# ga1i13o/DiffewS

Measured on AMD Instinct MI355X. Metric: few-shot episodes/sec (512x512, 1-shot, SD-2 UNet), higher is better.
Workload: dtype bf16; 1 GPU; SD-2.1 UNet + SD VAE, 512x512, 1-shot, 4 episodes/GPU/step (BASELINE.json configs[1]); nshot=1, resolution=512, parallelism=episode-sharded x1, hip_graph=True, residual_dtype=bf16, graph_owner=pipeline.run_episodes(captured=True)

## Files before the change

### diffews_amd/_lib.py

```python
import ctypes as C
import os

_HERE = os.path.dirname(os.path.abspath(__file__))
LIB_PATH = os.environ.get("DFW_LIB") or os.path.join(_HERE, "libdiffews_hip.so")

BF16, F16 = 0, 1
FILTER_BILINEAR, FILTER_BICUBIC = 0, 1
OUT_T, OUT_F32, OUT_NCHW_F32 = 0, 1, 2
ACT_NONE, ACT_SILU, ACT_CLAMP1 = 0, 1, 2

_vp, _i32, _i64, _f32, _sz = C.c_void_p, C.c_int32, C.c_int64, C.c_float, C.c_size_t


class GemmArgs(C.Structure):
    _fields_ = [("A", _vp), ("W", _vp), ("C", _vp), ("bias", _vp), ("rowbias", _vp), ("residual", _vp),
                ("workspace", _vp), ("workspace_bytes", _sz), ("a_elems", _i64), ("w_elems", _i64),
                ("M", _i32), ("N", _i32), ("K", _i32), ("lda", _i32), ("ldc", _i32), ("ldr", _i32), ("ld_rowbias", _i32),
                ("taps", _i32), ("Cin", _i32), ("Hi", _i32), ("Wi", _i32), ("Ho", _i32), ("Wo", _i32),
                ("stride", _i32), ("pad", _i32), ("ups", _i32), ("rows_per_img", _i32),
                ("out_scale", _f32), ("act", _i32), ("geglu", _i32), ("out_mode", _i32), ("splitk", _i32),
                ("batch", _i32), ("strideA", _i64), ("strideW", _i64), ("strideC", _i64), ("dtype", _i32),
                ("gn_partial", _vp), ("gn_groups", _i32),
                ("colscale", _f32), ("colscale_n", _i32), ("residual_f32", _i32), ("W_blocked", _vp)]


class FsaArgs(C.Structure):
    _fields_ = [("q", _vp), ("k", _vp), ("v", _vp), ("k_bank", _vp), ("v_bank", _vp), ("out", _vp),
                ("batch", _i32), ("heads", _i32), ("n_q", _i32), ("n_kv", _i32), ("n_bank", _i32), ("nshot", _i32),
                ("ldq", _i32), ("ldk", _i32), ("ldv", _i32), ("ldkb", _i32), ("ldvb", _i32), ("ldo", _i32),
                ("q_bs", _i64), ("k_bs", _i64), ("v_bs", _i64), ("kb_bs", _i64), ("vb_bs", _i64), ("o_bs", _i64),
                ("scale", _f32), ("dtype", _i32), ("n_plain", _i32), ("q_prescaled", _i32), ("lse", _vp),
                ("workspace", _vp), ("workspace_bytes", _sz), ("bank_shared", _i32)]


class XattnArgs(C.Structure):
    _fields_ = [("q", _vp), ("k", _vp), ("v", _vp), ("out", _vp),
                ("batch", _i32), ("heads", _i32), ("n_q", _i32), ("L", _i32),
                ("ldq", _i32), ("ldk", _i32), ("ldv", _i32), ("ldo", _i32),
                ("q_bs", _i64), ("k_bs", _i64), ("v_bs", _i64), ("o_bs", _i64),
                ("scale", _f32), ("dtype", _i32)]


class GroupNormArgs(C.Structure):
    _fields_ = [("x", _vp), ("y", _vp), ("gamma", _vp), ("beta", _vp), ("stats_ws", _vp), ("stats_ws_bytes", _sz),
                ("B", _i32), ("HW", _i32), ("C", _i32), ("groups", _i32), ("ldx", _i32), ("ldy", _i32),
                ("eps", _f32), ("silu", _i32), ("dtype", _i32), ("pre_partial", _vp), ("pre_chunks", _i32),
                ("x_f32", _i32)]


class LayerNormArgs(C.Structure):
    _fields_ = [("x", _vp), ("y", _vp), ("gamma", _vp), ("beta", _vp),
                ("rows", _i32), ("C", _i32), ("ldx", _i32), ("ldy", _i32), ("eps", _f32), ("dtype", _i32),
                ("x_f32", _i32)]


class ConvSmallArgs(C.Structure):
    _fields_ = [("x", _vp), ("W", _vp), ("bias", _vp), ("y", _vp),
                ("B", _i32), ("Cin", _i32), ("H", _i32), ("Wd", _i32), ("Cout", _i32), ("taps", _i32), ("ldy", _i32),
# ... 99 lines not shown
                ("q_bs", _i64), ("kv_bs", _i64), ("o_bs", _i64), ("dq_bs", _i64), ("dkv_bs", _i64),
                ("scale", _f32), ("dtype", _i32), ("workspace", _vp), ("workspace_bytes", _sz), ("delta_bytes", _sz)]


class VattnArgs(C.Structure):
    _fields_ = [("q", _vp), ("k", _vp), ("v", _vp), ("out", _vp),
                ("batch", _i32), ("n", _i32), ("head_dim", _i32), ("q_prescaled", _i32),
                ("ldq", _i32), ("ldk", _i32), ("ldv", _i32), ("ldo", _i32),
                ("q_bs", _i64), ("k_bs", _i64), ("v_bs", _i64), ("o_bs", _i64), ("dtype", _i32)]


class AdamWArgs(C.Structure):
    _fields_ = [("param", _vp), ("grad", _vp), ("exp_avg", _vp), ("exp_avg_sq", _vp), ("grad_sumsq", _vp), ("n", _i64),
                ("lr", _f32), ("beta1", _f32), ("beta2", _f32), ("eps", _f32), ("weight_decay", _f32), ("max_grad_norm", _f32),
                ("step", _i32), ("shadow", _vp), ("shadow_dtype", _i32), ("found_inf", _vp)]


class Config(C.Structure):
    _fields_ = [("conv_patch", _i32), ("big_kernels", _i32), ("big_bm", _i32), ("big_bn", _i32), ("big_bk", _i32),
                ("gemm_bm", _i32), ("gemm_bn", _i32), ("fsa_key_split", _i32),
                ("fsa_force_splits", _i32), ("big_min_tiles", _i32), ("k8", _i32)]


SYMBOLS = {
    "dfw_configure": (_i32, [C.POINTER(Config)]),
    "dfw_get_config": (None, [C.POINTER(Config)]),
    "dfw_version": (_i32, []),
    "dfw_error_string": (C.c_char_p, [_i32]),
    "dfw_graph_memset_nodes": (_i32, [_vp, C.POINTER(_i32)]),
    "dfw_gemm": (_i32, [C.POINTER(GemmArgs), _vp]),
    "dfw_gemm_workspace_bytes": (_sz, [C.POINTER(GemmArgs)]),
    "dfw_gemm_kernel_name": (_i32, [C.POINTER(GemmArgs), C.c_char_p, _sz]),
    "dfw_gemm_gn_chunks": (_i32, [C.POINTER(GemmArgs)]),
    "dfw_fsa_attention": (_i32, [C.POINTER(FsaArgs), _vp]),
    "dfw_fsa_workspace_bytes": (_sz, [C.POINTER(FsaArgs)]),
    "dfw_fsa_kernel_name": (_i32, [C.POINTER(FsaArgs), C.c_char_p, _sz]),
    "dfw_fsa_attention_sets": (_i32, [C.POINTER(FsaArgs), _i32, _vp]),
    "dfw_fsa_sets_kernel_name": (_i32, [C.POINTER(FsaArgs), _i32, C.c_char_p, _sz]),
    "dfw_fsa_attention_ragged": (_i32, [C.POINTER(FsaArgs), C.POINTER(_i32), _i32, _i32, _vp]),
    "dfw_fsa_ragged_kernel_name": (_i32, [C.POINTER(FsaArgs), C.POINTER(_i32), _i32, _i32, C.c_char_p, _sz]),
    "dfw_fsa_ragged_workspace_bytes": (_sz, [C.POINTER(FsaArgs), C.POINTER(_i32), _i32, _i32]),
    "dfw_fsa_attention_routed": (_i32, [C.POINTER(FsaArgs), _vp, C.POINTER(_i32), _i32, _i32, _vp]),
    "dfw_fsa_routed_kernel_name": (_i32, [C.POINTER(FsaArgs), _i32, _i32, C.c_char_p, _sz]),
    "dfw_fsa_routed_workspace_bytes": (_sz, [C.POINTER(FsaArgs), _i32, _i32]),
    "dfw_cross_attention": (_i32, [C.POINTER(XattnArgs), _vp]),
    "dfw_vae_attention": (_i32, [C.POINTER(VattnArgs), _vp]),
    "dfw_groupnorm": (_i32, [C.POINTER(GroupNormArgs), _vp]),
    "dfw_groupnorm_workspace_bytes": (_sz, [C.POINTER(GroupNormArgs)]),
    "dfw_layernorm": (_i32, [C.POINTER(LayerNormArgs), _vp]),
    "dfw_conv_small": (_i32, [C.POINTER(ConvSmallArgs), _vp]),
    "dfw_conv_small_gn_chunks": (_i32, [C.POINTER(ConvSmallArgs)]),
    "dfw_conv_small_kernel_name": (_i32, [C.POINTER(ConvSmallArgs), C.c_char_p, _sz]),
    "dfw_softmax_rows": (_i32, [_vp, _vp, _i64, _i32, _f32, _i32, _vp]),
    "dfw_softmax_groups": (_i32, [_vp, _vp, _i64, _i32, _i32, _i32, _i32, _vp]),
    "dfw_transpose": (_i32, [_vp, _vp, _i32, _i32, _i32, _i32, _vp]),
    "dfw_concat_channels": (_i32, [_vp, _vp, _vp, _i64, _i32, _i32, _i32, _vp]),
    "dfw_convert_f32": (_i32, [_vp, _vp, _i64, _i32, _vp]),
    "dfw_zero": (_i32, [_vp, _i64, _vp]),
    "dfw_split_f32": (_i32, [_vp, _vp, _vp, _i64, _i32, _vp]),
    "dfw_timestep_embedding": (_i32, [_vp, _vp, _i32, _i32, _i32, _f32, _i32, _vp]),
    "dfw_seg_postprocess": (_i32, [_vp, _vp, _vp, _vp, _vp, _i32, _i32, _i32, _f32, _vp]),
    "dfw_seg_postprocess_ex": (_i32, [_vp, _vp, _vp, _vp, _vp, _i32, _i32, _i32, _f32, _f32, _i32, _vp]),
    "dfw_seg_labels": (_i32, [_vp, _vp, _vp, _vp, _vp, _i32, _i32, _i32, _i32, _f32, _f32, _i32, _vp]),
    "dfw_seg_labels_cand": (_i32, [_vp, _vp, _vp, C.POINTER(_i32), _vp, _vp, _vp, _vp, _i32, _i32, _i32, _i32, _i32, _f32, _f32,
                                   _vp]),
    "dfw_meter_update": (_i32, [_vp, _vp, _vp, _vp, _i32, _i32, _vp]),
# ... 82 lines not shown
```

### diffews_amd/csrc/gemm8.hip

```cpp
#include "gemm_common.h"
#include <type_traits>

namespace dfw {

template <typename T, bool CONV, int BN>
__global__ __launch_bounds__(512, 2) void gemm8_kernel(const GemmP p) {
  constexpr int BM = 256, HT = 16384;
  constexpr bool N160 = BN == 160;
  static_assert(!(N160 && CONV), "the 256 x 160 tile is instantiated for Linear shapes only");
  constexpr int WH = BN / 128;
  constexpr int WGN = N160 ? 2 : BN / 64, WGM = 8 / WGN;
  constexpr int NBW = N160 ? 5 : 4;
  constexpr int WTM = BM / WGM, MB6 = WTM / 16, MH = MB6 / 2;
  constexpr int WDMA = N160 ? 3 : 2 * WH;
  constexpr int WB160 = 65536, WS160 = 24576;
  constexpr int STG = N160 ? WB160 + 2 * WS160 : (2 + WH) * 32768;
  extern __shared__ __attribute__((aligned(16))) char smem[];
  const int tid = threadIdx.x, lane = tid & 63;
  const int wave = __builtin_amdgcn_readfirstlane(tid >> 6);
  const int wr = wave >> 2;
  const int wm = wave / WGN, wc = wave % WGN;
  const uint32_t lds0 = lds_addr(smem);

  const int ntiles = p.ntm * p.ntn;
  const int nxb = gridDim.x >> 3, xcd = blockIdx.x & 7;
  const int Q = (ntiles + 7) >> 3;
  const int t_end = min(ntiles, (xcd + 1) * Q);
  const int tile0 = xcd * Q + (blockIdx.x >> 3);
  if (tile0 >= t_end) return;
  const int my_tiles = (t_end - tile0 + nxb - 1) / nxb;
  const int nkt = p.K >> 6;
  const int cpt = p.Cin >> 6;

  const int z = blockIdx.y;
  const char* Ab = p.A;
  const char* Wb = p.W;
  char* Cb = p.C;
  if (p.batch > 1) {
    Ab += (size_t)z * p.strideA * sizeof(T);
    Wb += (size_t)z * p.strideW * sizeof(T);
    Cb += (size_t)z * p.strideC * sizeof(T);
  }
  const u32x4 ra = make_srd(Ab, p.a_bytes);
  const u32x4 rw = make_srd(Wb, p.w_bytes);

  auto tile_coords = [&](int t) -> TileC {
    TileC c;
    const int tn = t % p.ntn, tm = t / p.ntn;
    c.m0 = tm * BM;
    c.n0 = tn * BN;
    c.img = 0; c.oy0 = 0; c.ox0 = 0;
    if constexpr (CONV) {
      c.img = tm / p.tpi;
      const int t2 = tm - c.img * p.tpi, tyi = t2 / p.tpr, txi = t2 - tyi * p.tpr;
      c.oy0 = tyi << 4;
      c.ox0 = txi << 4;
    }
    return c;
  };
  auto row_to_m = [&](const TileC& c, int r) -> int {
    if constexpr (CONV) return (c.img * p.Ho + c.oy0 + (r >> 4)) * p.Wo + c.ox0 + (r & 15);
    else return c.m0 + r;
  };

  const int lrow = lane >> 3;
  const int kc = (lane & 7) ^ ((((wave & 1) << 2) + (lane >> 4)) & 7);
  const unsigned limH = p.ups ? 2 * p.Hi : p.Hi, limW = p.ups ? 2 * p.Wi : p.Wi;
  const int ush = p.ups ? 1 : 0;
  int a_kt = 0, a_ti = 0;
  bool a_live = true;
  uint32_t a_v0 = 0;
  int a_m = 0, a_ix0 = 0;
  int a_iy0 = 0;
  uint32_t a_pix = 0;
  auto a_setup = [&](const TileC& c) {
    if constexpr (!CONV) {
      a_m = c.m0 + wave * 8 + lrow;
      a_v0 = (uint32_t)(((size_t)a_m * p.lda + kc * 8) * sizeof(T));
    } else {
      a_iy0 = (c.oy0 + (wave >> 1)) * p.stride - p.pad;
      a_ix0 = (c.ox0 + (wave & 1) * 8 + lrow) * p.stride - p.pad;
      a_pix = (uint32_t)c.img * (uint32_t)(p.Hi * p.Wi);
    }
  };
  auto a_advance = [&]() {
    if (++a_kt == nkt) {
      a_kt = 0;
      if (++a_ti < my_tiles) a_setup(tile_coords(tile0 + a_ti * nxb));
      else a_live = false;
    }
  };
  auto issue_a = [&](int buf) __attribute__((always_inline)) {
    int ky = 0, kx = 0, cc = 0;
    if constexpr (CONV) {
      cc = a_kt / 9;
      const int tap = a_kt - cc * 9;
      ky = tap / 3;
      kx = tap - ky * 3;
    }
#pragma unroll
    for (int h = 0; h < 2; ++h) {
      const uint32_t dst = lds0 + (uint32_t)(h * 32768 + buf * HT) + (uint32_t)wave * 1024u;
#pragma unroll
      for (int j = 0; j < 2; ++j) {
        uint32_t off;
        if constexpr (!CONV) {
          const int dr = h * 128 + j * 64;
          off = (a_m + dr < p.M && a_live) ? a_v0 + (uint32_t)dr * (uint32_t)p.lda * (uint32_t)sizeof(T) + (uint32_t)a_kt * 128u : kOOB;
        } else {
          int iy = a_iy0 + (h * 8 + j * 4) * p.stride + ky, ix = a_ix0 + kx;
          const bool ok = (unsigned)iy < limH && (unsigned)ix < limW && a_live;
          iy >>= ush;
          ix >>= ush;
          off = ok ? ((a_pix + (uint32_t)(iy * p.Wi + ix)) * (uint32_t)p.lda + (uint32_t)(cc * 64 + kc * 8)) * (uint32_t)sizeof(T) : kOOB;
        }
        dma16(ra, off, dst + j * 8192);
      }
    }
    a_advance();
  };
  int w_kt = 0, w_ti = 0;
  bool w_live = true;
  uint32_t w_v0 = 0;
  int w_n = 0;
  auto w_setup = [&](const TileC& c) {
    w_n = c.n0 + wave * 8 + lrow;
    w_v0 = (uint32_t)(((size_t)w_n * p.K + kc * 8) * sizeof(T));
  };
  auto issue_w = [&](int buf) __attribute__((always_inline)) {
    uint32_t koff = (uint32_t)w_kt * 128u;
    if constexpr (CONV) {
      const int cc = w_kt / 9, tap = w_kt - cc * 9;
      koff = (uint32_t)(tap * p.Cin + cc * 64) * (uint32_t)sizeof(T);
    }
    if constexpr (N160) {
      const uint32_t dst = lds0 + (uint32_t)(WB160 + buf * WS160) + (uint32_t)wave * 1024u;
#pragma unroll
      for (int j = 0; j < 3; ++j) {
        const uint32_t off = w_v0 + (uint32_t)(j * 64) * (uint32_t)p.K * (uint32_t)sizeof(T) + koff;
        const bool ok = w_live && (j < 2 || wave < 4);
        dma16(rw, ok ? off : kOOB, dst + j * 8192);
      }
    }
#pragma unroll
    for (int h = 0; h < (N160 ? 0 : WH); ++h) {
      const uint32_t dst = lds0 + (uint32_t)((2 + h) * 32768 + buf * HT) + (uint32_t)wave * 1024u;
#pragma unroll
      for (int j = 0; j < 2; ++j) {
        const uint32_t off = w_v0 + (uint32_t)(h * 128 + j * 64) * (uint32_t)p.K * (uint32_t)sizeof(T) + koff;
        bool ok = w_live;
        if constexpr (BN == 128) ok = ok && (w_n + j * 64 < p.N);
        dma16(rw, ok ? off : kOOB, dst + j * 8192);
      }
    }
    if (++w_kt == nkt) {
      w_kt = 0;
      if (++w_ti < my_tiles) {
        if (p.ntn > 1) w_setup(tile_coords(tile0 + w_ti * nxb));
      } else w_live = false;
    }
  };

  uint32_t ab0, ab1, wb0, wb1;
  {
    const int l15 = lane & 15, l4 = lane >> 4;
    const uint32_t fb = (uint32_t)(l15 * 128 + ((l4 ^ (l15 >> 1)) << 4));
    ab0 = (uint32_t)(wr * 32768 + (wm % (WGM / 2)) * WTM * 128) + fb;
    ab1 = ab0 ^ 64u;
    if constexpr (N160) wb0 = (uint32_t)(WB160 + wc * 80 * 128) + fb;
    else wb0 = (uint32_t)((2 + (wc >> 1)) * 32768 + (wc & 1) * 64 * 128) + fb;
    wb1 = wb0 ^ 64u;
  }
  const uint32_t wbase160 = wb0;

  f32x4 acc6[MB6][NBW];
  typename Tr<T>::v8 fa[MH][2], fw0[2][2], fw1[2][2], fw4[2];
  auto zero6 = [&]() __attribute__((always_inline)) {
#pragma unroll
    for (int i = 0; i < MB6; ++i)
#pragma unroll
      for (int j = 0; j < NBW; ++j) acc6[i][j] = f32x4{0.f, 0.f, 0.f, 0.f};
  };
  auto bar = [&]() __attribute__((always_inline)) {
    __builtin_amdgcn_sched_barrier(0);
    __builtin_amdgcn_s_barrier();
    asm volatile("" ::: "memory");
    __builtin_amdgcn_sched_barrier(0);
  };
  auto lgkm0 = [&]() __attribute__((always_inline)) {
    asm volatile("s_waitcnt lgkmcnt(0)" ::: "memory");
    __builtin_amdgcn_sched_barrier(0);
// ... 145 lines not shown
      if (p.gn_partial) {
        const int cp = lane & 31, rh = lane >> 5;
#pragma unroll
        for (int t = 0; t < 16; ++t) {
          const int r = rh * 16 + t;
          const uint32_t w2 = *(const uint32_t*)(stg + r * 128 + (((cp >> 2) ^ (r & 7)) << 4) + (cp & 3) * 4);
          typename Tr<T>::v4 pr = __builtin_bit_cast(typename Tr<T>::v4, i32x2{(int)w2, 0});
          const float a0 = (float)pr[0], a1 = (float)pr[1];
          gs0 += a0; gq0 += a0 * a0;
          gs1 += a1; gq1 += a1 * a1;
        }
      }
      const int c16 = lane & 7;
#pragma unroll
      for (int t = 0; t < 4; ++t) {
        const int r = (lane >> 3) + 8 * t;
        const int m2 = row_to_m(c, wm * WTM + i * 32 + r);
        const i32x4 val = *(const i32x4*)(stg + r * 128 + ((c16 ^ (r & 7)) << 4));
        if (m2 < p.M)
          *(i32x4*)(Cb + ((size_t)m2 * p.ldc + c.n0 + wc * 64 + c16 * 8) * sizeof(T)) = val;
      }
    }
    if (p.gn_partial) {
      float s2 = gs0 + gs1, q2 = gq0 + gq1;
      s2 += __shfl_xor(s2, 32, 64);
      q2 += __shfl_xor(q2, 32, 64);
      const int cpg = p.N / p.gn_groups, ppg = cpg >> 1;
      for (int o = 1; o < ppg; o <<= 1) {
        s2 += __shfl_xor(s2, o, 64);
        q2 += __shfl_xor(q2, o, 64);
      }
      const int cp = lane & 31;
      if (lane < 32 && (cp & (ppg - 1)) == 0) {
        const int tm = tile_id / p.ntn;
        const int chunk = (tm - c.img * p.tpi) * WGM + wm;
        const int grp = (c.n0 + wc * 64 + 2 * cp) / cpg;
        float* o2 = p.gn_partial + (((size_t)c.img * p.gn_chunks + chunk) * p.gn_groups + grp) * 2;
        o2[0] = s2;
        o2[1] = q2;
      }
    }
  };

  TileC ct = tile_coords(tile0);
  a_setup(ct);
  w_setup(ct);
  issue_w(0);
  issue_a(0);
  issue_w(1);
  wait_vm<WDMA>();
  bar();
  if (wr == 1) bar();
  zero6();
  int kt = 0, ti = 0, buf = 0;
  const int total = my_tiles * nkt;
#pragma unroll 1
  for (int g = 0; g < total; ++g) {
    read_a(0);
    read_w(fw0, 0);
    read_w(fw1, 1);
    if constexpr (N160) read_w4();
    issue_a(buf ^ 1);
    lgkm0();
    bar();
    __builtin_amdgcn_s_setprio(1);
    mfmas(0, 0, fw0);
    mfmas(0, 1, fw1);
    if constexpr (N160) mfmas4(0);
// ... 54 lines not shown
    (void)hipFuncSetAttribute((const void*)kfn, hipFuncAttributeMaxDynamicSharedMemorySize, (int)lds);
    hipLaunchKernelGGL(kfn, grid, dim3(512), lds, st, q);
  } else if constexpr (BN != 160) {
    auto kfn = gemm8_kernel<T, true, BN>;
    (void)hipFuncSetAttribute((const void*)kfn, hipFuncAttributeMaxDynamicSharedMemorySize, (int)lds);
    hipLaunchKernelGGL(kfn, grid, dim3(512), lds, st, q);
  } else {
    return DFW_ESHAPE;
  }
  DFW_CHECK_LAUNCH();
  return 0;
}

bool gemm8_eligible(const GemmP& p, int bn) {
  if (!cfg().k8 || p.out_mode != DFW_OUT_T || p.res_f32) return false;
  if ((p.K % 64) != 0 || (p.Cin % 64) != 0 || p.K / 64 < 2) return false;
  if (bn == 256) return (p.N % 256) == 0;
  return bn == 128 && (p.N % 64) == 0 && cfg().k8 >= 2;
}

bool gemm8_n160_eligible(const GemmP& p) {
  if (!cfg().k8 || !cfg().big_kernels || p.taps != 1 || p.out_mode != DFW_OUT_T || p.res_f32 || p.geglu || p.act != DFW_ACT_NONE) return false;
  if (p.batch > 1 || p.splitk > 1 || (p.N % 160) != 0 || (p.N % 128) == 0 || (p.K % 64) != 0 || p.K / 64 < 2) return false;
  if ((p.ldc % 8) != 0 || ((uintptr_t)p.C & 15)) return false;
  return (long long)((p.M + 255) / 256) * (p.N / 160) >= cfg().big_min_tiles;
}

int launch_gemm8(const GemmP& p, const GemmPlan& pl, hipStream_t st) {
  if (pl.bn == 160) return DFW_BY_DTYPE(p, launch8<T, 160>(p, pl, st));
  if (pl.bn == 256) return DFW_BY_DTYPE(p, launch8<T, 256>(p, pl, st));
  return DFW_BY_DTYPE(p, launch8<T, 128>(p, pl, st));
}

}
```

### diffews_amd/csrc/gemm_common.h

```cpp
#pragma once
#include "common.h"

namespace dfw {

struct GemmP {
  const char* A; const char* W; char* C;
  const char* Wblk;
  const float* bias; const float* rowbias; const char* residual; float* partial;
  uint32_t a_bytes, w_bytes;
  int M, N, K, lda, ldc, ldr, ldrb;
  int taps, Cin, Hi, Wi, Ho, Wo, stride, pad, ups, rows_per_img;
  float out_scale;
  float cs; int cs_n;
  int act, geglu, out_mode, splitk, batch;
  int res_f32;
  long long strideA, strideW, strideC;
  int nk, cpt, ntn, ntm;
  int plan_bm, plan_bn, dtype_bf16;
  float* gn_partial; int gn_groups, gn_chunks;
  int conv_chunk_major;
  int tw, tw_log2, tpr, tpi;
};

template <typename T, bool RF32 = false>
// ... 163 lines not shown
  }
  __device__ __forceinline__ void store(const GemmP& p, float* out, int n_w0, int lane) {
    const int cpg = p.N / p.gn_groups;
#pragma unroll
    for (int j = 0; j < 4; ++j) {
#pragma unroll
      for (int o = 1; o < 16; o <<= 1) {
        s[j] += __shfl_xor(s[j], o, 64);
        q[j] += __shfl_xor(q[j], o, 64);
      }
      if (cpg >= 8) { s[j] += __shfl_xor(s[j], 16, 64); q[j] += __shfl_xor(q[j], 16, 64); }
      if (cpg >= 16) { s[j] += __shfl_xor(s[j], 32, 64); q[j] += __shfl_xor(q[j], 32, 64); }
    }
    if (cpg >= 32) { s[0] += s[1]; q[0] += q[1]; s[2] += s[3]; q[2] += q[3]; }
    if (cpg >= 64) { s[0] += s[2]; q[0] += q[2]; }
    const int l15 = lane & 15, l4 = lane >> 4;
    if (l15 != 0) return;
    const int lstep = cpg >= 16 ? 4 : cpg / 4;
    if (l4 % lstep) return;
    const int jstep = cpg >= 64 ? 4 : (cpg >= 32 ? 2 : 1);
#pragma unroll
    for (int j = 0; j < 4; ++j) {
      if (j % jstep) continue;
      const int grp = (n_w0 + j * 16 + 4 * l4) / cpg;
      out[grp * 2] = s[j];
      out[grp * 2 + 1] = q[j];
    }
  }
};

struct TileC {
  int m0, n0;
  int img, oy0, ox0;
};

enum class GemmKernel { Tile, Big, K8, Patch, Patch8 };
struct GemmPlan {
  GemmKernel kernel;
  int bm, bn, bk, splitk;
  int gn_chunks;
  bool f32o, rf32;
};

#define DFW_BY_DTYPE(p, ...) \
  ((p).dtype_bf16 ? [&] { using T = __bf16; return __VA_ARGS__; }() : [&] { using T = _Float16; return __VA_ARGS__; }())

}
```

### diffews_amd/csrc/misc.hip

```cpp
#include "common.h"
#include <stdio.h>
#include <stdlib.h>

namespace dfw {

struct CsP {
  const float* x; const float* W; const float* bias; char* y;
  int B, Cin, H, Wd, Cout, taps, ldy, out_mode;
  float in_scale, out_scale;
  int iters;
  float* gn_partial; int gn_groups, gn_chunks;
  long long ybs;
  const float* x1; const float* x2; int b0, b1;
};

__device__ __forceinline__ const float* cs_image(const CsP& p, int b) {
  const size_t per = (size_t)p.Cin * p.H * p.Wd;
  if (p.x1 == nullptr || b < p.b0) return p.x + (size_t)b * per;
  if (b < p.b1) return p.x1 + (size_t)(b - p.b0) * per;
  return p.x2 + (size_t)(b - p.b1) * per;
}

template <typename T>
__global__ __launch_bounds__(256) void conv_small_kernel(const CsP p) {
// ... 888 lines not shown
        const int c = count_memset_nodes(child, total, depth + 1);
        if (c < 0) { free(nodes); return -1; }
        cnt += c;
      }
    }
  }
  free(nodes);
  return cnt;
}

extern "C" int dfw_graph_memset_nodes(void* graph, int32_t* n_nodes) {
  if (!graph) return DFW_EINVAL;
  if (n_nodes) *n_nodes = 0;
  const int c = count_memset_nodes((hipGraph_t)graph, n_nodes, 0);
  return c < 0 ? DFW_EINVAL : c;
}

static const dfw_config kDefaultCfg = {3, 1, 0, 0, 0, 0, 0, 1, 0, 192, 3};
static dfw_config g_cfg = kDefaultCfg;
namespace dfw { const dfw_config& cfg() { return g_cfg; } }

extern "C" int dfw_configure(const dfw_config* c) {
  if (!c) { g_cfg = kDefaultCfg; return 0; }
  if (c->conv_patch < 0 || c->conv_patch > 4 || c->fsa_force_splits < 0 || c->big_min_tiles < 1 || c->k8 < 0 || c->k8 > 3) return DFW_EINVAL;
  if (c->gemm_bm && !((c->gemm_bm == 128 && (c->gemm_bn == 128 || c->gemm_bn == 64)) || (c->gemm_bm == 64 && c->gemm_bn == 64))) return DFW_EINVAL;
  g_cfg = *c;
  return 0;
}

extern "C" void dfw_get_config(dfw_config* out) {
  if (out) *out = g_cfg;
}

extern "C" int dfw_version(void) { return 110; }

extern "C" const char* dfw_error_string(int code) {
  switch (code) {
    case 0: return "success";
    case DFW_EINVAL: return "invalid argument (null pointer or non-positive size)";
    case DFW_ESHAPE: return "shape not supported by the gfx950 kernel (alignment / multiple-of constraint)";
    case DFW_ERANGE: return "tensor exceeds the 2 GiB buffer-descriptor range";
    case DFW_EWORKSPACE: return "workspace missing or too small";
    default: return code > 0 ? hipGetErrorString((hipError_t)code) : "unknown error";
  }
}
```

### diffews_amd/ops.py

```python
import ctypes as C
import os
import math

import torch

from . import _lib as L

_DT = {torch.bfloat16: L.BF16, torch.float16: L.F16}


def _stream():
    return C.c_void_p(torch.cuda.current_stream().cuda_stream)


def _p(t):
    return C.c_void_p(t.data_ptr()) if t is not None else None


def _dt(t):
    try:
        return _DT[t.dtype]
    except KeyError:
        raise TypeError(f"engine storage dtype must be bfloat16 or float16, got {t.dtype}")

# ... 278 lines not shown
        gemm_hook("fsa_attention", 4.0 * heads * 64 * N * keys, e0, e1, (B, heads, N, keys))
        return out
    _fsa_routed_call(a, table.data_ptr(), host, nbank, min_shots)
    return out


def zeros(shape, dtype, device="cuda"):
    n = 1
    for d in shape:
        n *= int(d)
    esz = torch.empty(0, dtype=dtype).element_size()
    pad = (-(n * esz)) % 16 // esz if (n * esz) % 16 else 0
    buf = torch.empty(n + pad, dtype=dtype, device=device)
    L.check(L.lib().dfw_zero(buf.data_ptr(), (n + pad) * esz, _stream()), "dfw_zero")
    return buf[:n].view(*shape)


def split_storage(x, dtype):
    assert x.dtype == torch.float32 and x.is_contiguous() and x.numel() % 8 == 0
    hi = torch.empty(x.shape, dtype=dtype, device=x.device)
    lo = torch.empty(x.shape, dtype=dtype, device=x.device)
    L.check(L.lib().dfw_split_f32(x.data_ptr(), hi.data_ptr(), lo.data_ptr(), x.numel(), _DT[dtype], _stream()), "dfw_split_f32")
    return hi, lo


def linear_stream(x, w, bias=None, residual=None):
    if x.dtype != torch.float32:
        return linear(x, w, bias=bias, residual=residual)
    hi, lo = split_storage(x, w.dtype)
    y = linear(hi, w, bias=bias, residual=residual, out_f32=True)
    return linear(lo, w, residual=y, out_f32=True)


def conv3x3_stream(x, w, cout, bias=None, lo=True, **kw):
    if x.dtype != torch.float32:
        return conv3x3(x, w, cout, bias=bias, **kw)
    if not lo:
        return conv3x3(to_storage(x, w.dtype), w, cout, bias=bias, out_f32=True, **kw)
    hi, lo = split_storage(x, w.dtype)
    gn_groups = kw.pop("gn_groups", 0)
    y = conv3x3(hi, w, cout, bias=bias, out_f32=True, **kw)
    return conv3x3(lo, w, cout, residual=y, out_f32=True, gn_groups=gn_groups, **kw)


FSA_QSCALE = 64 ** -0.5 * math.log2(math.e)


VATTN_QSCALE = 512 ** -0.5 * math.log2(math.e)


def vae_attention(q, k, v, out=None):
    B, N, D = q.shape
    assert D == 512 and k.shape == q.shape and v.shape == q.shape and q.stride(2) == 1 and k.stride(2) == 1 and v.stride(2) == 1
    if out is None:
        out = torch.empty(B, N, D, dtype=q.dtype, device=q.device)
    a = L.VattnArgs()
    a.q, a.k, a.v, a.out = q.data_ptr(), k.data_ptr(), v.data_ptr(), out.data_ptr()
    a.batch, a.n, a.head_dim, a.q_prescaled = B, N, D, 1
    a.ldq, a.ldk, a.ldv, a.ldo = q.stride(1), k.stride(1), v.stride(1), out.stride(1)
    a.q_bs, a.k_bs, a.v_bs, a.o_bs = q.stride(0), k.stride(0), v.stride(0), out.stride(0)
    a.dtype = _dt(q)
    L.check(L.lib().dfw_vae_attention(C.byref(a), _stream()), "dfw_vae_attention")
    return out


def cross_attention(q, k, v, heads, scale=None):
    B, N, Cq = q.shape
    assert Cq == heads * 64 and q.stride(2) == 1 and k.stride(2) == 1 and v.stride(2) == 1
    out = torch.empty(B, N, Cq, dtype=q.dtype, device=q.device)
    a = L.XattnArgs()
    a.q, a.k, a.v, a.out = q.data_ptr(), k.data_ptr(), v.data_ptr(), out.data_ptr()
    a.batch, a.heads, a.n_q, a.L = B, heads, N, k.shape[1]
    a.ldq, a.ldk, a.ldv, a.ldo = q.stride(1), k.stride(1), v.stride(1), Cq
    a.q_bs, a.k_bs, a.v_bs, a.o_bs = q.stride(0), k.stride(0), v.stride(0), N * Cq
    a.scale = scale if scale is not None else 64 ** -0.5
# ... 365 lines not shown
```

### diffews_amd/packing.py

```python
import torch


def pack_conv3x3(w):
    co, ci = w.shape[:2]
    return w.permute(0, 2, 3, 1).reshape(co, 9 * ci).contiguous()


def block_conv3x3(wp):
    co, k = wp.shape
    ci = k // 9
    assert k == 9 * ci and ci % 32 == 0
    return wp.view(co, 9, ci // 32, 32).permute(1, 2, 0, 3).contiguous()


def pack_conv1x1(w):
    return w.reshape(w.shape[0], w.shape[1]).contiguous()


def pack_conv_small(w):
    co, ci, k, _ = w.shape
    return w.float().permute(0, 2, 3, 1).reshape(co, k * k, ci).contiguous()


def geglu_perm(n_half):
    assert n_half % 32 == 0
    t = torch.arange(n_half // 32)
    i = torch.arange(32)
    val = (t[:, None] * 32 + i[None, :])
    gate = val + n_half
    return torch.stack([val, gate], dim=1).reshape(-1)


def pack_geglu(w, b):
    perm = geglu_perm(w.shape[0] // 2)
    return w[perm].contiguous(), b.float()[perm].contiguous()


def pack_conv3x3_dgrad(w):
    co, ci, kh, kw = w.shape
    assert kh == 3 and kw == 3
    return w.flip(2, 3).permute(1, 2, 3, 0).reshape(ci, 9 * co).contiguous()


def unpack_conv3x3_grad(g):
    co, _, ci = g.shape
# ... 2 lines not shown
```

### diffews_amd/unet.py

```python
from dataclasses import dataclass

import os

import torch

from . import _lib as L
from . import ops, ops_bwd, packing, weights


@dataclass
class UNet2DConditionOutput:
    sample: torch.Tensor = None


class _Cfg(dict):
    __getattr__ = dict.__getitem__


def _resolve_device(d):
    d = torch.device(d)
    if d.type == "cuda" and d.index is None:
        d = torch.device("cuda", torch.cuda.current_device() if torch.cuda.is_available() else 0)
    return d

# ... 333 lines not shown
            att = ops.fsa_attention(q, k, v, heads, k[:n_ref], v[:n_ref], nshot=n_ref // bq, n_plain=n_ref,
                                    q_prescaled=True)
        elif self.k_bank is None:
            self.k_bank, self.v_bank = k, v
            att = ops.fsa_attention(q, k, v, heads, q_prescaled=True)
        else:
            bank_b = self.k_bank.shape[0]
            if bank_b % B != 0:
                raise ValueError(f"bank holds {bank_b} support images, not a multiple of the query batch {B}")
            att = ops.fsa_attention(q, k, v, heads, self.k_bank, self.v_bank, nshot=bank_b // B, q_prescaled=True)
        t = ops.linear(att.view(-1, C), self.w_o1, bias=self.b_o1, residual=t, out_f32=f32s)
        ln = ops.layernorm(t, *self.ln[1], out_dtype=dt)
        if isinstance(ehs2d, tuple) and len(ehs2d) == 3 and ehs2d[2] and self.fold2 is not None:
            G, Ut, Lf = self.fold2
            sc = ops.linear(ln, G, out_f32=True)
            pr = ops.softmax_groups(sc, heads, Lf, dt)
            t = ops.linear(pr, Ut, bias=self.b_o2, residual=t, out_f32=f32s)
        else:
            q2 = ops.linear(ln, self.w_q2).view(B, N, C)
            o, kv_all = self.kv_slice[0], ehs2d
            if isinstance(kv_all, tuple):
                kv2 = kv_all[1].view(B, L_ctx, -1)[..., o:o + 2 * C]
            else:
                kv2 = ops.linear(ehs2d, self.w_kv2).view(B, L_ctx, 2 * C)
            ca = ops.cross_attention(q2, kv2[..., :C], kv2[..., C:], heads)
            t = ops.linear(ca.view(-1, C), self.w_o2, bias=self.b_o2, residual=t, out_f32=f32s)
        ln = ops.layernorm(t, *self.ln[2], out_dtype=dt)
        ff = ops.linear(ln, self.w_ff1, bias=self.b_ff1, geglu=True)
        t = ops.linear(ff, self.w_ff2, bias=self.b_ff2, residual=t, out_f32=f32s)
        return ops.linear_stream(t, self.w_out, bias=self.b_out, residual=x.view(-1, C)).view(B, H, W, C)


class _Conv:
    def __init__(self, sd, p, dev, dt):
        self.w = packing.pack_conv3x3(sd[p + "weight"]).to(dev, dt)
        self.b = sd[p + "bias"].float().to(dev)
        self.cout = sd[p + "weight"].shape[0]


class MyUNet2DConditionModel:

    def __init__(self, config=None, state_dict=None, torch_dtype=torch.bfloat16, device="cuda", residual_dtype=None,
                 **kwargs):
        cfg = weights.default_unet_config()
        cfg.update(config or {})
        cfg.update(kwargs)
        self.config = _Cfg(cfg)
        if residual_dtype not in (None, torch_dtype, torch.float32):
            raise ValueError("residual_dtype must be None (= torch_dtype) or torch.float32")
        self.residual_dtype = residual_dtype or torch_dtype
        self._f32s = self.residual_dtype == torch.float32
        if torch_dtype not in (torch.bfloat16, torch.float16):
            raise ValueError(
                "engine storage dtype must be torch.bfloat16 or torch.float16: the MI355X path keeps activations in 16 bits "
                "(fp32 accumulation, statistics and boundary tensors).  The reference launcher's default is fp32 "
                "(evaluation_util/main_oss.py:335-336): pass --half_precision / torch_dtype=torch.float16 -- z0 then sits "
                "1.5e-3 (relative L2) from the fp32 path, see DESIGN.md section 4")
        self.dtype = torch_dtype
        self.device = torch.device(device)
        L.lib()
        if state_dict is None:
            raise ValueError("MyUNet2DConditionModel needs a state_dict (use from_pretrained / synthetic weights)")
        weights.check_state_dict(state_dict, weights.unet_param_shapes(cfg), "unet")
        self._build(state_dict)

    @classmethod
    def from_pretrained(cls, path, subfolder=None, revision=None, torch_dtype=torch.bfloat16, device="cuda",
                        residual_dtype=None, **kw):
# ... 372 lines not shown
```

### diffews_amd/vae.py

```python
import torch

from . import _lib as L
from . import ops, packing, weights
from .unet import _Cfg, _Conv, _needs_rebuild


class _VaeResnet:
    def __init__(self, sd, p, dev, dt, groups):
        g = lambda k: sd[p + k]
        self.groups = groups
        self.g1, self.b1 = g("norm1.weight").float().to(dev), g("norm1.bias").float().to(dev)
        self.g2, self.b2 = g("norm2.weight").float().to(dev), g("norm2.bias").float().to(dev)
        self.cout = g("conv1.weight").shape[0]
        self.w1 = packing.pack_conv3x3(g("conv1.weight")).to(dev, dt)
        self.cb1 = g("conv1.bias").float().to(dev)
        self.w2 = packing.pack_conv3x3(g("conv2.weight")).to(dev, dt)
        self.cb2 = g("conv2.bias").float().to(dev)
        self.ws = None
        if p + "conv_shortcut.weight" in sd:
            self.ws = packing.pack_conv1x1(g("conv_shortcut.weight")).to(dev, dt)
            self.bs = g("conv_shortcut.bias").float().to(dev)

    def __call__(self, x):
        B, H, W, Cin = x.shape
# ... 72 lines not shown

    @torch.no_grad()
    def __call__(self, x):
        if isinstance(x, (list, tuple)):
            x = [t.to(dtype=torch.float32).contiguous() for t in x]
        else:
            x = x.to(dtype=torch.float32).contiguous()
        h = ops.conv_small(x, self.w_in, self.b_in, self.c0, 9, self.dt, gn_groups=self.groups, out_f32=self.f32s)
        for lvl, (res, down) in enumerate(self.blocks):
            for r in res:
                h = r(h)
            if down is not None:
                h = ops.conv3x3_stream(h, down.w, down.cout, bias=down.b, stride=2, pad=0, gn_groups=self.groups,
                                       lo=lvl >= self.single_round_levels)
        h = self.mid(h)
        h = ops.groupnorm(h, *self.gn_out, self.groups, 1e-6, silu=True, out_dtype=self.dt)
        co = self.conv_out
        return ops.conv3x3(h, co.w, co.cout, bias=co.b, out_nchw_f32=True)


class _Decoder:
    def __init__(self, vae, sd):
        cfg, dev, dt, g = vae.config, vae.device, vae.dtype, vae.config["norm_num_groups"]
        self.dt, self.groups, self.f32s = dt, g, (vae.residual_dtype == torch.float32 and vae.decoder_f32_stream)
        boc, lpb = list(cfg["block_out_channels"]), cfg["layers_per_block"]
        rboc = boc[::-1]
        self.c0 = rboc[0]
        self.w_in = packing.pack_conv_small(sd["decoder.conv_in.weight"]).to(dev)
        self.b_in = sd["decoder.conv_in.bias"].float().to(dev)
        self.mid = _Mid(sd, "decoder.mid_block.", dev, dt, g)
        self.blocks = []
        for i in range(len(boc)):
            res = [_VaeResnet(sd, f"decoder.up_blocks.{i}.resnets.{j}.", dev, dt, g) for j in range(lpb + 1)]
            up = _Conv(sd, f"decoder.up_blocks.{i}.upsamplers.0.conv.", dev, dt) if i != len(boc) - 1 else None
            self.blocks.append((res, up))
        self.gn_out = (sd["decoder.conv_norm_out.weight"].float().to(dev),
                       sd["decoder.conv_norm_out.bias"].float().to(dev))
        self.conv_out = _Conv(sd, "decoder.conv_out.", dev, dt)

    @torch.no_grad()
    def __call__(self, z, clamp=False):
        z = z.to(dtype=torch.float32).contiguous()
        h = ops.conv_small(z, self.w_in, self.b_in, self.c0, 9, self.dt, gn_groups=self.groups, out_f32=self.f32s)
        h = self.mid(h)
        for res, up in self.blocks:
            for r in res:
                h = r(h)
            if up is not None:
                h = ops.conv3x3_stream(h, up.w, up.cout, bias=up.b, ups=True, gn_groups=self.groups)
        h = ops.groupnorm(h, *self.gn_out, self.groups, 1e-6, silu=True, out_dtype=self.dt)
        co = self.conv_out
        return ops.conv3x3(h, co.w, co.cout, bias=co.b, out_nchw_f32=True,
                           act=L.ACT_CLAMP1 if clamp else L.ACT_NONE)


class _Conv1x1Boundary:

    def __init__(self, sd, p, dev, dt):
        self.w = packing.pack_conv_small(sd[p + "weight"]).to(dev)
        self.b = sd[p + "bias"].float().to(dev)
        self.cout, self.dt = sd[p + "weight"].shape[0], dt
        self._head = {}

    @torch.no_grad()
    def __call__(self, x, in_scale=1.0, out_scale=1.0, out=None, channels=None):
        w, b, cout = self.w, self.b, self.cout
        if channels is not None and channels != cout:
            if channels not in self._head:
                self._head[channels] = (w[:channels].contiguous(), b[:channels].contiguous())
            (w, b), cout = self._head[channels], channels
        return ops.conv_small(x.to(dtype=torch.float32).contiguous(), w, b, cout, 1, self.dt,
                              nchw_f32_out=True, in_scale=in_scale, out_scale=out_scale, out=out)


class _DiagonalGaussian:
    def __init__(self, moments):
        self.mean, self.logvar = torch.chunk(moments, 2, dim=1)
        self.logvar = self.logvar.clamp(-30.0, 20.0)

    def mode(self):
        return self.mean

# ... 77 lines not shown
```

### include/diffews_hip.h

```cpp
#ifndef DIFFEWS_HIP_H
#define DIFFEWS_HIP_H

#include <stddef.h>
#include <stdint.h>

#ifdef __cplusplus
extern "C" {
#endif

typedef void* dfw_stream_t;

enum { DFW_BF16 = 0, DFW_F16 = 1 };
enum { DFW_OUT_T = 0, DFW_OUT_F32 = 1, DFW_OUT_NCHW_F32 = 2 };
enum { DFW_ACT_NONE = 0, DFW_ACT_SILU = 1, DFW_ACT_CLAMP1 = 2  };
enum {
  DFW_EINVAL = -1,
  DFW_ESHAPE = -2,
  DFW_ERANGE = -3,
  DFW_EWORKSPACE = -4
};

int dfw_version(void);
const char* dfw_error_string(int code);

// ... 6 lines not shown
  int32_t fsa_force_splits;
  int32_t big_min_tiles;
  int32_t k8;
} dfw_config;
int dfw_configure(const dfw_config* cfg);
void dfw_get_config(dfw_config* out);

int dfw_graph_memset_nodes(void* hip_graph, int32_t* n_nodes);

typedef struct {
  const void* A; const void* W; void* C;
  const float* bias; const float* rowbias; const void* residual;
  void* workspace; size_t workspace_bytes;
  int64_t a_elems, w_elems;
  int32_t M, N, K;
  int32_t lda, ldc, ldr;
  int32_t ld_rowbias;
  int32_t taps, Cin, Hi, Wi, Ho, Wo, stride, pad, ups;
  int32_t rows_per_img;
  float out_scale;
  int32_t act, geglu, out_mode, splitk;
  int32_t batch; int64_t strideA, strideW, strideC;
  int32_t dtype;
  float* gn_partial; int32_t gn_groups;
  float colscale; int32_t colscale_n;
  int32_t residual_f32;
  const void* W_blocked;
} dfw_gemm_args;

int dfw_gemm(const dfw_gemm_args* a, dfw_stream_t stream);
size_t dfw_gemm_workspace_bytes(const dfw_gemm_args* a);
int dfw_gemm_kernel_name(const dfw_gemm_args* a, char* buf, size_t n);
int32_t dfw_gemm_gn_chunks(const dfw_gemm_args* a);

typedef struct {
  const void* q; const void* k; const void* v;
  const void* k_bank; const void* v_bank; void* out;
  int32_t batch, heads, n_q, n_kv, n_bank, nshot;
  int32_t ldq, ldk, ldv, ldkb, ldvb, ldo;
  int64_t q_bs, k_bs, v_bs, kb_bs, vb_bs, o_bs;
  float scale;
  int32_t dtype;
  int32_t n_plain;
  int32_t q_prescaled;
  float* lse;
  void* workspace; size_t workspace_bytes;
  int32_t bank_shared;
} dfw_fsa_args;

int dfw_fsa_attention(const dfw_fsa_args* a, dfw_stream_t stream);
size_t dfw_fsa_workspace_bytes(const dfw_fsa_args* a);
int dfw_fsa_kernel_name(const dfw_fsa_args* a, char* buf, size_t n);
int dfw_fsa_attention_sets(const dfw_fsa_args* a, int32_t group, dfw_stream_t stream);
int dfw_fsa_sets_kernel_name(const dfw_fsa_args* a, int32_t group, char* buf, size_t n);
int dfw_fsa_attention_ragged(const dfw_fsa_args* a, const int32_t* shots, int32_t nsets, int32_t group, dfw_stream_t stream);
int dfw_fsa_ragged_kernel_name(const dfw_fsa_args* a, const int32_t* shots, int32_t nsets, int32_t group, char* buf, size_t n);
size_t dfw_fsa_ragged_workspace_bytes(const dfw_fsa_args* a, const int32_t* shots, int32_t nsets, int32_t group);
int dfw_fsa_attention_routed(const dfw_fsa_args* a, const int32_t* table, const int32_t* table_host, int32_t nbank,
                             int32_t min_shots, dfw_stream_t stream);
int dfw_fsa_routed_kernel_name(const dfw_fsa_args* a, int32_t nbank, int32_t min_shots, char* buf, size_t n);
size_t dfw_fsa_routed_workspace_bytes(const dfw_fsa_args* a, int32_t nbank, int32_t min_shots);

typedef struct {
  const void* q; const void* k; const void* v; void* out;
  int32_t batch, heads, n_q, L;
  int32_t ldq, ldk, ldv, ldo;
// ... 360 lines not shown
```

Before: 100.9 episodes/s.

## Fold nearest-neighbor 2x upsample into a 2x2 sub-pixel conv for VAE upsamplers

Adds a new conv mode to the gemm8 kernel in which the nearest-upsample plus 3x3 conv is rewritten as four parity-specific 2x2 convolutions over the un-upsampled input. The folded weights are precomputed at load time. This cuts the K dimension from 9*Cin to 4*Cin per output pixel, removing redundant multiply-accumulates on duplicated pixels in the VAE decoder upsamplers. It adds a new weight buffer, new tile/parity indexing and GroupNorm partial-chunk bookkeeping. Folded weights are summed in fp32 and then rounded, so outputs can differ slightly numerically.

```diff
diff --git a/diffews_amd/_lib.py b/diffews_amd/_lib.py
--- a/diffews_amd/_lib.py
+++ b/diffews_amd/_lib.py
@@ -24,6 +24,12 @@
                 ("colscale", _f32), ("colscale_n", _i32), ("residual_f32", _i32), ("W_blocked", _vp)]
 
 
+class ConvUp2xArgs(C.Structure):
+    _fields_ = [("x", _vp), ("W", _vp), ("y", _vp), ("bias", _vp), ("x_elems", _i64), ("w_elems", _i64),
+                ("B", _i32), ("Hi", _i32), ("Wi", _i32), ("Cin", _i32), ("Cout", _i32), ("ldx", _i32), ("ldy", _i32),
+                ("dtype", _i32), ("gn_partial", _vp), ("gn_groups", _i32)]
+
+
 class FsaArgs(C.Structure):
     _fields_ = [("q", _vp), ("k", _vp), ("v", _vp), ("k_bank", _vp), ("v_bank", _vp), ("out", _vp),
                 ("batch", _i32), ("heads", _i32), ("n_q", _i32), ("n_kv", _i32), ("n_bank", _i32), ("nshot", _i32),
@@ -189,6 +195,9 @@
     "dfw_gemm_workspace_bytes": (_sz, [C.POINTER(GemmArgs)]),
     "dfw_gemm_kernel_name": (_i32, [C.POINTER(GemmArgs), C.c_char_p, _sz]),
     "dfw_gemm_gn_chunks": (_i32, [C.POINTER(GemmArgs)]),
+    "dfw_conv_up2x": (_i32, [C.POINTER(ConvUp2xArgs), _vp]),
+    "dfw_conv_up2x_kernel_name": (_i32, [C.POINTER(ConvUp2xArgs), C.c_char_p, _sz]),
+    "dfw_conv_up2x_gn_chunks": (_i32, [C.POINTER(ConvUp2xArgs)]),
     "dfw_fsa_attention": (_i32, [C.POINTER(FsaArgs), _vp]),
     "dfw_fsa_workspace_bytes": (_sz, [C.POINTER(FsaArgs)]),
     "dfw_fsa_kernel_name": (_i32, [C.POINTER(FsaArgs), C.c_char_p, _sz]),
diff --git a/diffews_amd/csrc/gemm8.hip b/diffews_amd/csrc/gemm8.hip
--- a/diffews_amd/csrc/gemm8.hip
+++ b/diffews_amd/csrc/gemm8.hip
@@ -3,9 +3,11 @@
 
 namespace dfw {
 
-template <typename T, bool CONV, int BN>
+template <typename T, bool CONV, int BN, bool UP2X = false>
 __global__ __launch_bounds__(512, 2) void gemm8_kernel(const GemmP p) {
   constexpr int BM = 256, HT = 16384;
+  static_assert(!UP2X || (CONV && BN != 160), "the folded upsample conv is a conv mode of the 256 / 128 wide tiles");
+  constexpr int KW = UP2X ? 4 : 1;
   constexpr bool N160 = BN == 160;
   static_assert(!(N160 && CONV), "the 256 x 160 tile is instantiated for Linear shapes only");
   constexpr int WH = BN / 128;
@@ -46,6 +48,11 @@
 
   auto tile_coords = [&](int t) -> TileC {
     TileC c;
+    c.par = 0;
+    if constexpr (UP2X) {
+      c.par = t & 3;
+      t >>= 2;
+    }
     const int tn = t % p.ntn, tm = t / p.ntn;
     c.m0 = tm * BM;
     c.n0 = tn * BN;
@@ -59,7 +66,8 @@
     return c;
   };
   auto row_to_m = [&](const TileC& c, int r) -> int {
-    if constexpr (CONV) return (c.img * p.Ho + c.oy0 + (r >> 4)) * p.Wo + c.ox0 + (r & 15);
+    if constexpr (UP2X) return (c.img * p.Ho + 2 * (c.oy0 + (r >> 4)) + (c.par >> 1)) * p.Wo + 2 * (c.ox0 + (r & 15)) + (c.par & 1);
+    else if constexpr (CONV) return (c.img * p.Ho + c.oy0 + (r >> 4)) * p.Wo + c.ox0 + (r & 15);
     else return c.m0 + r;
   };
 
@@ -81,6 +89,10 @@
       a_iy0 = (c.oy0 + (wave >> 1)) * p.stride - p.pad;
       a_ix0 = (c.ox0 + (wave & 1) * 8 + lrow) * p.stride - p.pad;
       a_pix = (uint32_t)c.img * (uint32_t)(p.Hi * p.Wi);
+      if constexpr (UP2X) {
+        a_iy0 += c.par >> 1;
+        a_ix0 += c.par & 1;
+      }
     }
   };
   auto a_advance = [&]() {
@@ -92,7 +104,11 @@
   };
   auto issue_a = [&](int buf) __attribute__((always_inline)) {
     int ky = 0, kx = 0, cc = 0;
-    if constexpr (CONV) {
+    if constexpr (UP2X) {
+      cc = a_kt >> 2;
+      ky = (a_kt >> 1) & 1;
+      kx = a_kt & 1;
+    } else if constexpr (CONV) {
       cc = a_kt / 9;
       const int tap = a_kt - cc * 9;
       ky = tap / 3;
@@ -122,14 +138,18 @@
   int w_kt = 0, w_ti = 0;
   bool w_live = true;
   uint32_t w_v0 = 0;
-  int w_n = 0;
+  int w_n = 0, w_par = 0;
   auto w_setup = [&](const TileC& c) {
     w_n = c.n0 + wave * 8 + lrow;
-    w_v0 = (uint32_t)(((size_t)w_n * p.K + kc * 8) * sizeof(T));
+    w_par = c.par;
+    w_v0 = (uint32_t)(((size_t)w_n * p.K * KW + kc * 8) * sizeof(T));
   };
   auto issue_w = [&](int buf) __attribute__((always_inline)) {
     uint32_t koff = (uint32_t)w_kt * 128u;
-    if constexpr (CONV) {
+    if constexpr (UP2X) {
+      const int cc = w_kt >> 2, tap = w_kt & 3;
+      koff = (uint32_t)((w_par * 4 + tap) * p.Cin + cc * 64) * (uint32_t)sizeof(T);
+    } else if constexpr (CONV) {
       const int cc = w_kt / 9, tap = w_kt - cc * 9;
       koff = (uint32_t)(tap * p.Cin + cc * 64) * (uint32_t)sizeof(T);
     }
@@ -147,7 +167,7 @@
       const uint32_t dst = lds0 + (uint32_t)((2 + h) * 32768 + buf * HT) + (uint32_t)wave * 1024u;
 #pragma unroll
       for (int j = 0; j < 2; ++j) {
-        const uint32_t off = w_v0 + (uint32_t)(h * 128 + j * 64) * (uint32_t)p.K * (uint32_t)sizeof(T) + koff;
+        const uint32_t off = w_v0 + (uint32_t)(h * 128 + j * 64) * (uint32_t)(p.K * KW) * (uint32_t)sizeof(T) + koff;
         bool ok = w_live;
         if constexpr (BN == 128) ok = ok && (w_n + j * 64 < p.N);
         dma16(rw, ok ? off : kOOB, dst + j * 8192);
@@ -156,7 +176,7 @@
     if (++w_kt == nkt) {
       w_kt = 0;
       if (++w_ti < my_tiles) {
-        if (p.ntn > 1) w_setup(tile_coords(tile0 + w_ti * nxb));
+        if (UP2X || p.ntn > 1) w_setup(tile_coords(tile0 + w_ti * nxb));
       } else w_live = false;
     }
   };
@@ -368,8 +388,8 @@
       }
       const int cp = lane & 31;
       if (lane < 32 && (cp & (ppg - 1)) == 0) {
-        const int tm = tile_id / p.ntn;
-        const int chunk = (tm - c.img * p.tpi) * WGM + wm;
+        const int tm = (UP2X ? tile_id >> 2 : tile_id) / p.ntn;
+        const int chunk = ((tm - c.img * p.tpi) * KW + c.par) * WGM + wm;
         const int grp = (c.n0 + wc * 64 + 2 * cp) / cpg;
         float* o2 = p.gn_partial + (((size_t)c.img * p.gn_chunks + chunk) * p.gn_groups + grp) * 2;
         o2[0] = s2;
@@ -490,4 +510,92 @@
   return DFW_BY_DTYPE(p, launch8<T, 128>(p, pl, st));
 }
 
-}
+template <typename T, int BN>
+static int launch_up2x(const GemmP& p, hipStream_t st) {
+  constexpr size_t lds = (size_t)(2 + BN / 128) * 32768 + 32768;
+  int nwg = p.ntm * p.ntn;
+  if (nwg > 256) nwg = 256;
+  nwg = (nwg + 7) & ~7;
+  auto kfn = gemm8_kernel<T, true, BN, true>;
+  (void)hipFuncSetAttribute((const void*)kfn, hipFuncAttributeMaxDynamicSharedMemorySize, (int)lds);
+  hipLaunchKernelGGL(kfn, dim3(nwg), dim3(512), lds, st, p);
+  DFW_CHECK_LAUNCH();
+  return 0;
+}
+
+static int up2x_gn_chunks(const dfw_conv_up2x_args* a, int bn) {
+  if (a->gn_groups <= 0 || (a->Cout % a->gn_groups) != 0) return 0;
+  const int cpg = a->Cout / a->gn_groups;
+  if (cpg < 4 || cpg > 64 || (cpg & (cpg - 1))) return 0;
+  return 4 * (a->Hi / 16) * (a->Wi / 16) * (8 / (bn / 64));
+}
+
+static int up2x_plan(const dfw_conv_up2x_args* a, int& bn) {
+  if (!a || !a->x || !a->W || !a->y) return DFW_EINVAL;
+  if (a->B <= 0 || a->Hi <= 0 || a->Wi <= 0 || a->Cin <= 0 || a->Cout <= 0 || a->x_elems <= 0 || a->w_elems <= 0) return DFW_EINVAL;
+  if (a->dtype != DFW_BF16 && a->dtype != DFW_F16) return DFW_EINVAL;
+  if (a->gn_groups < 0 || (a->gn_partial && a->gn_groups == 0)) return DFW_EINVAL;
+  if ((a->Hi % 16) != 0 || (a->Wi % 16) != 0 || (a->Cin % 64) != 0 || (a->Cout % 64) != 0) return DFW_ESHAPE;
+  if (a->ldx < a->Cin || (a->ldx % 8) != 0 || a->ldy < a->Cout || (a->ldy % 8) != 0) return DFW_ESHAPE;
+  if (((uintptr_t)a->x & 15) || ((uintptr_t)a->W & 15) || ((uintptr_t)a->y & 15)) return DFW_ESHAPE;
+  if ((a->bias && ((uintptr_t)a->bias & 15)) || (a->gn_partial && ((uintptr_t)a->gn_partial & 3))) return DFW_ESHAPE;
+  const int64_t pix = (int64_t)a->B * a->Hi * a->Wi;
+  if (a->x_elems * 2 >= (1ll << 31) || a->w_elems * 2 >= (1ll << 31) || 4 * pix >= (1ll << 31)) return DFW_ERANGE;
+  if (a->x_elems < pix * a->ldx - (a->ldx - a->Cin) || a->w_elems < (int64_t)a->Cout * 16 * a->Cin) return DFW_EINVAL;
+  bn = (a->Cout % 256) == 0 ? 256 : 128;
+  if (a->gn_partial && up2x_gn_chunks(a, bn) == 0) return DFW_ESHAPE;
+  return 0;
+}
+
+}
+
+using namespace dfw;
+
+extern "C" int dfw_conv_up2x_kernel_name(const dfw_conv_up2x_args* a, char* buf, size_t n) {
+  if (!buf || n == 0) return DFW_EINVAL;
+  buf[0] = 0;
+  int bn = 0;
+  const int rc = up2x_plan(a, bn);
+  if (rc) return rc;
+  snprintf(buf, n, "gemm8_kernel<%s,256,%d,64,up2x>", a->dtype == DFW_BF16 ? "bf16" : "f16", bn);
+  return 0;
+}
+
+extern "C" int32_t dfw_conv_up2x_gn_chunks(const dfw_conv_up2x_args* a) {
+  int bn = 0;
+  if (!a) return 0;
+  dfw_conv_up2x_args q = *a;
+  q.gn_partial = nullptr;
+  return up2x_plan(&q, bn) ? 0 : up2x_gn_chunks(&q, bn);
+}
+
+extern "C" int dfw_conv_up2x(const dfw_conv_up2x_args* a, dfw_stream_t stream) {
+  int bn = 0;
+  const int rc = up2x_plan(a, bn);
+  if (rc) return rc;
+  GemmP p = {};
+  p.A = (const char*)a->x; p.W = (const char*)a->W; p.C = (char*)a->y;
+  p.bias = a->bias;
+  p.a_bytes = (uint32_t)(a->x_elems * 2);
+  p.w_bytes = (uint32_t)(a->w_elems * 2);
+  p.Hi = a->Hi; p.Wi = a->Wi; p.Ho = 2 * a->Hi; p.Wo = 2 * a->Wi;
+  p.M = a->B * p.Ho * p.Wo; p.N = a->Cout; p.K = 4 * a->Cin;
+  p.lda = a->ldx; p.ldc = a->ldy;
+  p.taps = 4; p.Cin = a->Cin; p.stride = 1; p.pad = 1; p.ups = 0;
+  p.rows_per_img = p.Ho * p.Wo;
+  p.out_scale = 1.0f; p.out_mode = DFW_OUT_T; p.splitk = 1; p.batch = 1;
+  p.nk = p.K / 64; p.cpt = a->Cin / 64;
+  p.dtype_bf16 = a->dtype == DFW_BF16;
+  p.tw = 16; p.tw_log2 = 4;
+  p.tpr = a->Wi / 16;
+  p.tpi = p.tpr * (a->Hi / 16);
+  p.ntm = 4 * a->B * p.tpi;
+  p.ntn = (a->Cout + bn - 1) / bn;
+  if (a->gn_partial) {
+    p.gn_partial = a->gn_partial; p.gn_groups = a->gn_groups;
+    p.gn_chunks = up2x_gn_chunks(a, bn);
+  }
+  hipStream_t st = (hipStream_t)stream;
+  if (bn == 256) return DFW_BY_DTYPE(p, launch_up2x<T, 256>(p, st));
+  return DFW_BY_DTYPE(p, launch_up2x<T, 128>(p, st));
+}
diff --git a/diffews_amd/csrc/gemm_common.h b/diffews_amd/csrc/gemm_common.h
--- a/diffews_amd/csrc/gemm_common.h
+++ b/diffews_amd/csrc/gemm_common.h
@@ -219,6 +219,7 @@
 struct TileC {
   int m0, n0;
   int img, oy0, ox0;
+  int par;
 };
 
 enum class GemmKernel { Tile, Big, K8, Patch, Patch8 };
diff --git a/diffews_amd/csrc/misc.hip b/diffews_amd/csrc/misc.hip
--- a/diffews_amd/csrc/misc.hip
+++ b/diffews_amd/csrc/misc.hip
@@ -944,7 +944,7 @@
   if (out) *out = g_cfg;
 }
 
-extern "C" int dfw_version(void) { return 110; }
+extern "C" int dfw_version(void) { return 111; }
 
 extern "C" const char* dfw_error_string(int code) {
   switch (code) {
diff --git a/diffews_amd/ops.py b/diffews_amd/ops.py
--- a/diffews_amd/ops.py
+++ b/diffews_amd/ops.py
@@ -334,8 +334,12 @@
     return linear(lo, w, residual=y, out_f32=True)
 
 
-def conv3x3_stream(x, w, cout, bias=None, lo=True, **kw):
+def conv3x3_stream(x, w, cout, bias=None, lo=True, w_up2x=None, **kw):
     if x.dtype != torch.float32:
+        if w_up2x is not None and UP2X_FOLD and kw.get("ups") and set(kw) <= {"ups", "gn_groups"}:
+            y = conv3x3_up2x(x, w_up2x, cout, bias=bias, gn_groups=kw.get("gn_groups", 0))
+            if y is not None:
+                return y
         return conv3x3(x, w, cout, bias=bias, **kw)
     if not lo:
         return conv3x3(to_storage(x, w.dtype), w, cout, bias=bias, out_f32=True, **kw)
@@ -343,6 +347,48 @@
     gn_groups = kw.pop("gn_groups", 0)
     y = conv3x3(hi, w, cout, bias=bias, out_f32=True, **kw)
     return conv3x3(lo, w, cout, residual=y, out_f32=True, gn_groups=gn_groups, **kw)
+
+
+UP2X_FOLD = True
+
+
+def conv3x3_up2x(x, w_folded, cout, bias=None, gn_groups=0):
+    assert x.dim() == 4 and x.is_contiguous()
+    B, Hi, Wi, Cin = x.shape
+    assert w_folded.shape == (cout, 16 * Cin) and w_folded.dtype == x.dtype and w_folded.is_contiguous()
+    out = torch.empty(B, 2 * Hi, 2 * Wi, cout, dtype=x.dtype, device=x.device)
+    a = L.ConvUp2xArgs()
+    a.x, a.W, a.y = x.data_ptr(), w_folded.data_ptr(), out.data_ptr()
+    a.bias = _p(_f32(bias, "bias"))
+    a.x_elems, a.w_elems = x.numel(), w_folded.numel()
+    a.B, a.Hi, a.Wi, a.Cin, a.Cout, a.ldx, a.ldy = B, Hi, Wi, Cin, cout, Cin, cout
+    a.dtype = _dt(x)
+    lib = L.lib()
+    name = C.create_string_buffer(64)
+    rc = lib.dfw_conv_up2x_kernel_name(C.byref(a), name, 64)
+    if rc == -2:
+        return None
+    L.check(rc, "dfw_conv_up2x_kernel_name")
+    stats = None
+    if gn_groups:
+        a.gn_groups = gn_groups
+        chunks = lib.dfw_conv_up2x_gn_chunks(C.byref(a))
+        if chunks > 0:
+            part = torch.empty(B, chunks, gn_groups, 2, dtype=torch.float32, device=x.device)
+            a.gn_partial = part.data_ptr()
+            stats = (part, chunks, gn_groups)
+    if gemm_hook is not None:
+        e0, e1 = torch.cuda.Event(enable_timing=True), torch.cuda.Event(enable_timing=True)
+        e0.record()
+        L.check(lib.dfw_conv_up2x(C.byref(a), _stream()), "dfw_conv_up2x")
+        e1.record()
+        M = B * 4 * Hi * Wi
+        gemm_hook(name.value.decode(), 2.0 * M * cout * 4 * Cin, e0, e1, (M, cout, 4 * Cin, 4, 1, 1, 1, 1))
+    else:
+        L.check(lib.dfw_conv_up2x(C.byref(a), _stream()), "dfw_conv_up2x")
+    if stats is not None:
+        out._gn_stats = stats
+    return out
 
 
 FSA_QSCALE = 64 ** -0.5 * math.log2(math.e)
diff --git a/diffews_amd/packing.py b/diffews_amd/packing.py
--- a/diffews_amd/packing.py
+++ b/diffews_amd/packing.py
@@ -11,6 +11,25 @@
     ci = k // 9
     assert k == 9 * ci and ci % 32 == 0
     return wp.view(co, 9, ci // 32, 32).permute(1, 2, 0, 3).contiguous()
+
+
+UP2X_TAPS = (((0,), (1, 2)), ((0, 1), (2,)))
+
+
+def fold_up2x(wp, dtype=None):
+    co, k = wp.shape
+    ci = k // 9
+    assert k == 9 * ci
+    w = (wp if wp.dtype == torch.float64 else wp.float()).view(co, 3, 3, ci)
+    out = torch.zeros(co, 2, 2, 2, 2, ci, dtype=w.dtype, device=wp.device)
+    for py in range(2):
+        for px in range(2):
+            for ty in range(2):
+                for tx in range(2):
+                    for ky in UP2X_TAPS[py][ty]:
+                        for kx in UP2X_TAPS[px][tx]:
+                            out[:, py, px, ty, tx] += w[:, ky, kx]
+    return out.reshape(co, 16 * ci).to(dtype if dtype is not None else wp.dtype).contiguous()
 
 
 def pack_conv1x1(w):
diff --git a/diffews_amd/unet.py b/diffews_amd/unet.py
--- a/diffews_amd/unet.py
+++ b/diffews_amd/unet.py
@@ -389,8 +389,10 @@
 
 
 class _Conv:
-    def __init__(self, sd, p, dev, dt):
-        self.w = packing.pack_conv3x3(sd[p + "weight"]).to(dev, dt)
+    def __init__(self, sd, p, dev, dt, up2x=False):
+        wp = packing.pack_conv3x3(sd[p + "weight"])
+        self.w = wp.to(dev, dt)
+        self.wf = packing.fold_up2x(wp, dt).to(dev) if up2x else None
         self.b = sd[p + "bias"].float().to(dev)
         self.cout = sd[p + "weight"].shape[0]
 
diff --git a/diffews_amd/vae.py b/diffews_amd/vae.py
--- a/diffews_amd/vae.py
+++ b/diffews_amd/vae.py
@@ -128,7 +128,7 @@
         self.blocks = []
         for i in range(len(boc)):
             res = [_VaeResnet(sd, f"decoder.up_blocks.{i}.resnets.{j}.", dev, dt, g) for j in range(lpb + 1)]
-            up = _Conv(sd, f"decoder.up_blocks.{i}.upsamplers.0.conv.", dev, dt) if i != len(boc) - 1 else None
+            up = _Conv(sd, f"decoder.up_blocks.{i}.upsamplers.0.conv.", dev, dt, up2x=True) if i != len(boc) - 1 else None
             self.blocks.append((res, up))
         self.gn_out = (sd["decoder.conv_norm_out.weight"].float().to(dev),
                        sd["decoder.conv_norm_out.bias"].float().to(dev))
@@ -143,7 +143,7 @@
             for r in res:
                 h = r(h)
             if up is not None:
-                h = ops.conv3x3_stream(h, up.w, up.cout, bias=up.b, ups=True, gn_groups=self.groups)
+                h = ops.conv3x3_stream(h, up.w, up.cout, bias=up.b, ups=True, gn_groups=self.groups, w_up2x=up.wf)
         h = ops.groupnorm(h, *self.gn_out, self.groups, 1e-6, silu=True, out_dtype=self.dt)
         co = self.conv_out
         return ops.conv3x3(h, co.w, co.cout, bias=co.b, out_nchw_f32=True,
diff --git a/include/diffews_hip.h b/include/diffews_hip.h
--- a/include/diffews_hip.h
+++ b/include/diffews_hip.h
@@ -62,6 +62,19 @@
 size_t dfw_gemm_workspace_bytes(const dfw_gemm_args* a);
 int dfw_gemm_kernel_name(const dfw_gemm_args* a, char* buf, size_t n);
 int32_t dfw_gemm_gn_chunks(const dfw_gemm_args* a);
+
+typedef struct {
+  const void* x; const void* W; void* y; const float* bias;
+  int64_t x_elems, w_elems;
+  int32_t B, Hi, Wi, Cin, Cout;
+  int32_t ldx, ldy;
+  int32_t dtype;
+  float* gn_partial; int32_t gn_groups;
+} dfw_conv_up2x_args;
+
+int dfw_conv_up2x(const dfw_conv_up2x_args* a, dfw_stream_t stream);
+int dfw_conv_up2x_kernel_name(const dfw_conv_up2x_args* a, char* buf, size_t n);
+int32_t dfw_conv_up2x_gn_chunks(const dfw_conv_up2x_args* a);
 
 typedef struct {
   const void* q; const void* k; const void* v;
```

After: 103.6 episodes/s, median of 6. 2.7% higher.
